# zrjer/Sparse-Matrix-Factorization-Library

Hardware: AMD Instinct MI355X
Metric: numeric-factorization GFLOP/s (supernodal Cholesky) (higher is better)
Workload: dtype f64; 1 GPU; 3D 7-point Laplacian 128^3 SPD Cholesky fp64, geometric ND, devSlotSize 8694792192; n=2097152, nnz_input=8339456, nsuper=35419, factor_doubles=3787034536, parallelism=single GPU, grid_rule=BASELINE config

## Files before the change

sparse-matrix-factorization-library_amd/csrc/sf_kernels.hip:

```cpp
#include "sf_kernels.h"
#include <cstdlib>
#include "sf_panel.h"
#include "sf_wave.h"

namespace sf {

__device__ __forceinline__ int lower_bound_i32(const int32_t* __restrict__ a, int n, int32_t key) {
    int lo = 0, hi = n;
    while (lo < hi) {
        const int mid = (lo + hi) >> 1;
        if (a[mid] < key) lo = mid + 1; else hi = mid;
    }
    return lo;
}

__global__ void __launch_bounds__(256)
k_load_panels(const int64_t* __restrict__ Lp, const int32_t* __restrict__ Li, const double* __restrict__ Lx, int32_t n,
              const int32_t* __restrict__ Super, const int32_t* __restrict__ SuperMap,
              const int64_t* __restrict__ Lsip, const int32_t* __restrict__ Lsi,
              const int64_t* __restrict__ Lsxp, double* __restrict__ Lsx, int skip_diag,
              const int8_t* __restrict__ load_mask) {
    const int32_t j = blockIdx.x * blockDim.x + threadIdx.x;
    if (j >= n) return;
    const int32_t s = SuperMap[j];
    if (load_mask && !load_mask[s]) return;
    const int32_t c0 = Super[s], c1 = Super[s + 1];
    const int64_t r0 = Lsip[s];
    const int32_t nsrow = (int32_t)(Lsip[s + 1] - r0);
    const int32_t nscol = c1 - c0;
    double* col = Lsx + Lsxp[s] + (int64_t)(j - c0) * nsrow;
    const int32_t* below = Lsi + r0 + nscol;
    for (int64_t p = Lp[j]; p < Lp[j + 1]; ++p) {
        const int32_t i = Li[p];
        if (skip_diag && i == j) continue;
        const int32_t si = (i < c1) ? (i - c0) : nscol + lower_bound_i32(below, nsrow - nscol, i);
        col[si] = Lx[p];
    }
}

__global__ void __launch_bounds__(256)
k_build_loadmap(const int64_t* __restrict__ Lp, const int32_t* __restrict__ Li, int32_t n,
                const int32_t* __restrict__ Super, const int32_t* __restrict__ SuperMap,
                const int64_t* __restrict__ Lsip, const int32_t* __restrict__ Lsi,
                const int64_t* __restrict__ Lsxp, int64_t base, int skip_diag, int64_t* __restrict__ map) {
    const int32_t j = blockIdx.x * blockDim.x + threadIdx.x;
    if (j >= n) return;
    const int32_t s = SuperMap[j];
    const int32_t c0 = Super[s], c1 = Super[s + 1];
    const int64_t r0 = Lsip[s];
    const int32_t nsrow = (int32_t)(Lsip[s + 1] - r0);
    const int32_t nscol = c1 - c0;
    const int64_t col = base + Lsxp[s] + (int64_t)(j - c0) * nsrow;
    const int32_t* below = Lsi + r0 + nscol;
    for (int64_t p = Lp[j]; p < Lp[j + 1]; ++p) {
        const int32_t i = Li[p];
        if (skip_diag && i == j) { map[p] = -1; continue; }
        const int32_t si = (i < c1) ? (i - c0) : nscol + lower_bound_i32(below, nsrow - nscol, i);
        map[p] = col + si;
    }
}

__global__ void __launch_bounds__(256)
k_load_mapped(const double* __restrict__ Lx, const int64_t* __restrict__ map, int64_t nnz, double* __restrict__ Lsx) {
    for (int64_t p = (int64_t)blockIdx.x * blockDim.x + threadIdx.x; p < nnz; p += (int64_t)gridDim.x * blockDim.x) {
        const int64_t m = map[p];
        if (m >= 0) Lsx[m] = Lx[p];
    }
}

__global__ void __launch_bounds__(256)
k_loadmap_drop(const int64_t* __restrict__ drop, int64_t count, int64_t* __restrict__ map) {
    for (int64_t k = (int64_t)blockIdx.x * blockDim.x + threadIdx.x; k < count; k += (int64_t)gridDim.x * blockDim.x) map[drop[k]] = -1;
}

void launch_loadmap_drop(const int64_t* drop, int64_t count, int64_t* map, hipStream_t st) {
    if (count <= 0) return;
    const int64_t blocks = std::min<int64_t>((count + 255) / 256, 1024);
    hipLaunchKernelGGL(k_loadmap_drop, dim3((unsigned)blocks), dim3(256), 0, st, drop, count, map);
}

void launch_build_loadmap(const int64_t* Lp, const int32_t* Li, int32_t n, const int32_t* Super, const int32_t* SuperMap,
                          const int64_t* Lsip, const int32_t* Lsi, const int64_t* Lsxp, int64_t base, int skip_diag, int64_t* map, hipStream_t st) {
    if (n <= 0) return;
    hipLaunchKernelGGL(k_build_loadmap, dim3((n + 255) / 256), dim3(256), 0, st, Lp, Li, n, Super, SuperMap, Lsip, Lsi, Lsxp, base, skip_diag, map);
}

void launch_load_mapped(const double* Lx, const int64_t* map, int64_t nnz, double* Lsx, hipStream_t st) {
    if (nnz <= 0) return;
    const int64_t blocks = std::min<int64_t>((nnz + 255) / 256, 256 * 16);
    hipLaunchKernelGGL(k_load_mapped, dim3((unsigned)blocks), dim3(256), 0, st, Lx, map, nnz, Lsx);
}

void launch_load_panels(const int64_t* Lp, const int32_t* Li, const double* Lx, int32_t n,
                        const int32_t* Super, const int32_t* SuperMap, const int64_t* Lsip, const int32_t* Lsi,
                        const int64_t* Lsxp, double* Lsx, int skip_diag, const int8_t* load_mask, hipStream_t st) {
    if (n <= 0) return;
    hipLaunchKernelGGL(k_load_panels, dim3((n + 255) / 256), dim3(256), 0, st,
                       Lp, Li, Lx, n, Super, SuperMap, Lsip, Lsi, Lsxp, Lsx, skip_diag, load_mask);
}

template <int W>
__device__ __forceinline__ void potrf_block_w(const PotrfTask& t, double* __restrict__ Lsx, int* __restrict__ info) {
    double* A = Lsx + t.panel + t.diag + (int64_t)t.diag * t.ld;
    const int b = t.b;
    const int lane = threadIdx.x;
    const int64_t ld = t.ld;

    double a[W];
#pragma unroll
    for (int c = 0; c < W; ++c) {
        double v = (c == lane) ? 1.0 : 0.0;
        if (lane < b && c <= lane) v = A[lane + c * ld];
        a[c] = v;
    }
    bool bad = false;
    double dnext = a[0];
#pragma unroll
    for (int j = 0; j < W; ++j) {
        const double djj = readlane_f64(dnext, j);
        bad = bad || !(djj > 0.0);
        const double rinv = rsqrt_full(djj);
        const double lj = a[j] * rinv;
        a[j] = lj;
        if (j + 1 < W) dnext = __builtin_fma(-lj, lj, a[j + 1]);
#pragma unroll
        for (int c = j + 1; c < W; ++c) a[c] = __builtin_fma(-lj, readlane_f64(lj, c), a[c]);
    }
    if (bad && lane == 0) atomicOr(info, 1);
#pragma unroll
    for (int c = 0; c < W; ++c)
        if (lane < b && c <= lane) A[lane + c * ld] = a[c];
}

__global__ void __launch_bounds__(64)
k_potrf_block(const PotrfTask* __restrict__ tasks, double* __restrict__ Lsx, int* __restrict__ info) {
    const PotrfTask t = tasks[blockIdx.x];
    if (t.b <= 8) potrf_block_w<8>(t, Lsx, info);
    else if (t.b <= 16) potrf_block_w<16>(t, Lsx, info);
    else if (t.b <= 32) potrf_block_w<32>(t, Lsx, info);
    else potrf_block_w<NB>(t, Lsx, info);
}

void launch_potrf(const PotrfTask* tasks, int ntasks, double* Lsx, int* info, hipStream_t st) {
    if (ntasks <= 0) return;
    hipLaunchKernelGGL(k_potrf_block, dim3(ntasks), dim3(64), 0, st, tasks, Lsx, info);
}

template <int W>
__device__ __forceinline__ void getrf_block_w(const PotrfTask& t, double* __restrict__ Lsx, int64_t u_shift, int* __restrict__ info, const PivotCtl& pc) {
    double* PLd = Lsx + t.panel + t.diag + (int64_t)t.diag * t.ld;
    double* PUd = PLd + u_shift;
    const int b = t.b;
    const int lane = threadIdx.x;
    const int64_t ld = t.ld;

    double a[W];
#pragma unroll
    for (int c = 0; c < W; ++c) {
        double v = (c == lane) ? 1.0 : 0.0;
        if (lane < b && c < b) v = (c < lane) ? PLd[lane + c * ld] : PUd[c + lane * ld];
        a[c] = v;
    }
    bool bad = false, active = lane < b;
    int np = 0, pos = lane;
    getrf_panel_wave<false, W>(a, lane, 0, b, pc.tol, pc.eps, bad, np, pos, active, nullptr);
    if (bad && lane == 0) atomicOr(info, 1);
    if (np > 0 && lane == 0) atomicAdd(pc.nperturb, np);
#pragma unroll
    for (int c = 0; c < W; ++c) {
        if (lane < b && c < b) {
            if (c < pos) PLd[pos + c * ld] = a[c]; else PUd[c + pos * ld] = a[c];
        }
    }
    if (pc.pivpos && lane < b) {
        const int g0 = t.first_col + t.diag;
        pc.pivpos[g0 + lane] = g0 + pos;
        pc.pivinv[g0 + pos] = g0 + lane;
    }
}

__global__ void __launch_bounds__(64)
k_getrf_block(const PotrfTask* __restrict__ tasks, double* __restrict__ Lsx, int64_t u_shift, int* __restrict__ info, PivotCtl pc) {
    const PotrfTask t = tasks[blockIdx.x];
    if (t.b <= 8) getrf_block_w<8>(t, Lsx, u_shift, info, pc);
    else if (t.b <= 16) getrf_block_w<16>(t, Lsx, u_shift, info, pc);
    else if (t.b <= 32) getrf_block_w<32>(t, Lsx, u_shift, info, pc);
    else getrf_block_w<NB>(t, Lsx, u_shift, info, pc);
}

void launch_getrf(const PotrfTask* tasks, int ntasks, double* Lsx, int64_t u_shift, int* info, PivotCtl pc, hipStream_t st) {
    if (ntasks <= 0) return;
    hipLaunchKernelGGL(k_getrf_block, dim3(ntasks), dim3(64), 0, st, tasks, Lsx, u_shift, info, pc);
}

__global__ void __launch_bounds__(256)
k_pack_lu(const int32_t* __restrict__ Super, const int64_t* __restrict__ Lsip, const int64_t* __restrict__ Xp,
          const int64_t* __restrict__ RefXp, int32_t nsuper, const double* __restrict__ PL, const double* __restrict__ PU,
          double* __restrict__ out, int64_t e_begin, int64_t e_end) {
    for (int64_t e = e_begin + (int64_t)blockIdx.x * blockDim.x + threadIdx.x; e < e_end; e += (int64_t)gridDim.x * blockDim.x) {
        double* __restrict__ dst = out + (e - e_begin);
        int lo = 0, hi = nsuper;
        while (hi - lo > 1) {
            const int mid = (lo + hi) >> 1;
            if (RefXp[mid] <= e) lo = mid; else hi = mid;
        }
        const int s = lo;
        if (Xp[s] < 0) { *dst = 0.0; continue; }
        const int64_t nscol = Super[s + 1] - Super[s], nsrow = Lsip[s + 1] - Lsip[s];
        const int64_t lda = 2 * nsrow - nscol;
        const int64_t off = e - RefXp[s];
        const int64_t j = off / lda, R = off % lda;
        const double* pl = PL + Xp[s] + j * nsrow;
        double v;
        if (R < nscol) v = (R > j) ? pl[R] : PU[Xp[s] + j + R * nsrow];
        else if (R < nsrow) v = pl[R];
        else v = PU[Xp[s] + (R - nsrow + nscol) + j * nsrow];
        *dst = v;
    }
}

void launch_pack_lu(const int32_t* Super, const int64_t* Lsip, const int64_t* Xp, const int64_t* RefXp, int32_t nsuper,
                    const double* PL, const double* PU, double* out, int64_t e_begin, int64_t e_end, hipStream_t st) {
    if (e_end <= e_begin) return;
    const int64_t blocks = (e_end - e_begin + 255) / 256;
    hipLaunchKernelGGL(k_pack_lu, dim3((unsigned)(blocks < 65536 ? blocks : 65536)), dim3(256), 0, st,
                       Super, Lsip, Xp, RefXp, nsuper, PL, PU, out, e_begin, e_end);
}

__global__ void __launch_bounds__(256)
k_factor_hash(const int32_t* __restrict__ Super, const int64_t* __restrict__ Lsip, const int64_t* __restrict__ Xp,
              const int64_t* __restrict__ RefXp, int32_t nsuper, const double* __restrict__ PL, const double* __restrict__ PU, int lu,
              int64_t total, int64_t chunk, unsigned long long* __restrict__ H) {
    const int64_t begin = (int64_t)blockIdx.x * chunk, end = min(begin + chunk, total);
    if (begin >= end) return;
    const bool idle = begin + threadIdx.x >= end;
    int64_t e = idle ? end - 1 : begin + threadIdx.x;
    int lo = 0, hi = nsuper;
    while (hi - lo > 1) {
        const int mid = (lo + hi) >> 1;
        if (RefXp[mid] <= e) lo = mid; else hi = mid;
    }
    int s = lo;
    unsigned long long acc = 0;
    int64_t s_end = RefXp[s + 1], s_beg = RefXp[s], xp = Xp[s];
    int64_t nscol = Super[s + 1] - Super[s], nsrow = Lsip[s + 1] - Lsip[s];
    if (idle) e = end;
    for (; e < end; e += 256) {
        if (e >= s_end) {
            if (acc) atomicAdd(&H[s], acc);
            acc = 0;
            while (e >= RefXp[s + 1]) ++s;
            s_end = RefXp[s + 1]; s_beg = RefXp[s]; xp = Xp[s];
            nscol = Super[s + 1] - Super[s]; nsrow = Lsip[s + 1] - Lsip[s];
        }
        if (xp < 0) {
            e += ((s_end - e + 255) / 256 - 1) * 256;
            continue;
        }
        const int64_t off = e - s_beg;
        double v;
        if (!lu) {
            v = PL[xp + off];
        } else {
            const int64_t lda = 2 * nsrow - nscol;
            const int64_t j = off / lda, R = off % lda;
            if (R < nscol) v = (R > j) ? PL[xp + j * nsrow + R] : PU[xp + j + R * nsrow];
            else if (R < nsrow) v = PL[xp + j * nsrow + R];
            else v = PU[xp + (R - nsrow + nscol) + j * nsrow];
        }
        acc += (unsigned long long)__double_as_longlong(v) * ((2ull * (unsigned long long)e + 1ull) * 0x9E3779B97F4A7C15ull);
    }
    __shared__ int s_first;
    __shared__ unsigned long long s_part[4];
    if (threadIdx.x == 0) s_first = s;
    __syncthreads();
    const bool uniform = __syncthreads_and(s == s_first) != 0;
    if (!uniform) { if (acc) atomicAdd(&H[s], acc); return; }
    for (int off = 32; off > 0; off >>= 1) acc += __shfl_down(acc, off, 64);
    if ((threadIdx.x & 63) == 0) s_part[threadIdx.x >> 6] = acc;
    __syncthreads();
    if (threadIdx.x == 0) {
        const unsigned long long tot = s_part[0] + s_part[1] + s_part[2] + s_part[3];
        if (tot) atomicAdd(&H[s], tot);
    }
}

void launch_factor_hash(const int32_t* Super, const int64_t* Lsip, const int64_t* Xp, const int64_t* RefXp, int32_t nsuper,
                        const double* PL, const double* PU, int lu, int64_t total, unsigned long long* H, hipStream_t st) {
    if (total <= 0 || nsuper <= 0) return;
    const int64_t chunk = 256 * 64;
    const int64_t blocks = (total + chunk - 1) / chunk;
    hipLaunchKernelGGL(k_factor_hash, dim3((unsigned)blocks), dim3(256), 0, st, Super, Lsip, Xp, RefXp, nsuper, PL, PU, lu, total, chunk, H);
}

__global__ void __launch_bounds__(256)
k_lu_fill_u11(const FillTile* __restrict__ tiles, double* __restrict__ PL, const double* __restrict__ PU) {
    __shared__ double tile[64][65];
    const FillTile t = tiles[blockIdx.x];
    const int tx = threadIdx.x & 63, ty = threadIdx.x >> 6;
    const int jlo = max(t.c0, t.cb), jhi = min(t.c0 + 64, t.ce);
    {
        const int j = t.c0 + tx;
        for (int rr = ty; rr < 64; rr += 4) {
            const int R = t.r0 + rr;
            if (j >= jlo && j < jhi && R <= j) tile[rr][tx] = PU[t.xp + j + (int64_t)R * t.nsrow];
        }
    }
    __syncthreads();
    {
        const int R = t.r0 + tx;
        for (int jj = ty; jj < 64; jj += 4) {
            const int j = t.c0 + jj;
            if (j >= jlo && j < jhi && R <= j) PL[t.xp + R + (int64_t)j * t.nsrow] = tile[tx][jj];
        }
    }
}

void launch_lu_fill_u11(const FillTile* tiles, int64_t ntiles, double* PL, const double* PU, hipStream_t st) {
    if (ntiles <= 0) return;
    hipLaunchKernelGGL(k_lu_fill_u11, dim3((unsigned)ntiles), dim3(256), 0, st, tiles, PL, PU);
}

__global__ void __launch_bounds__(TRSM_ROWS)
k_trsm_block(const TrsmTask* __restrict__ tasks, double* __restrict__ Lsx, const int32_t* __restrict__ pivinv) {
    __shared__ __attribute__((aligned(16))) double Dt[NB][NB];
    __shared__ double Dinv[NB];
    const TrsmTask t = tasks[blockIdx.x];
    const double* Dg = Lsx + t.dpanel + t.diag + (int64_t)t.diag * t.ld;
    const int b = t.b;
    const int tid = threadIdx.x;

    for (int e = tid; e < b * NB; e += (int)blockDim.x) {
        const int k = e / NB, j = e % NB;
        Dt[k][j] = (j < b && k < j) ? Dg[j + (int64_t)k * t.ld] : 0.0;
    }
    if (tid < NB) Dinv[tid] = (tid < b && !t.unit) ? 1.0 / Dg[tid + (int64_t)tid * t.ld] : 1.0;
    __syncthreads();

    if (tid >= t.nrows) return;
    double* X = Lsx + t.panel + t.row0 + tid + (int64_t)t.diag * t.ld;
    const int64_t ld = t.ld;
    if (pivinv && t.unit) {
        const int g0 = t.first_col + t.diag;
        const int32_t* pv = pivinv + g0;
        double tmp[NB];
#pragma unroll
        for (int c = 0; c < NB; ++c) tmp[c] = X[(int64_t)(pv[min(c, b - 1)] - g0) * ld];
#pragma unroll
        for (int c = 0; c < NB; ++c)
            if (c < b) X[(int64_t)c * ld] = tmp[c];
    }

    for (int jb = 0; jb < b; jb += 8) {
        double acc[8];
#pragma unroll
        for (int u = 0; u < 8; ++u) acc[u] = X[min(jb + u, b - 1) * ld];
#pragma unroll
        for (int u = 0; u < 8; ++u) acc[u] = (jb + u < b) ? acc[u] : 0.0;
        for (int k0 = 0; k0 < jb; k0 += 8) {
            double xk[8];
#pragma unroll
            for (int v = 0; v < 8; ++v) xk[v] = X[(k0 + v) * ld];
#pragma unroll
            for (int v = 0; v < 8; ++v)
#pragma unroll
                for (int u = 0; u < 8; ++u) acc[u] -= xk[v] * Dt[k0 + v][jb + u];
        }
#pragma unroll
        for (int u = 0; u < 8; ++u) {
#pragma unroll
            for (int v = 0; v < u; ++v) acc[u] -= acc[v] * Dt[jb + v][jb + u];
            acc[u] *= Dinv[jb + u];
        }
#pragma unroll
        for (int u = 0; u < 8; ++u)
            if (jb + u < b) X[(jb + u) * ld] = acc[u];
    }
}

void launch_trsm(const TrsmTask* tasks, int ntasks, double* Lsx, const int32_t* pivinv, hipStream_t st) {
    if (ntasks <= 0) return;
    hipLaunchKernelGGL(k_trsm_block, dim3(ntasks), dim3(TRSM_ROWS), 0, st, tasks, Lsx, pivinv);
}

constexpr int LDS_LD = GEMM_BM + 16;
constexpr int GEMM_SK = GEMM_BK / 2;
#ifndef SF_GEMM_MIN_UNITS_DEFAULT
#define SF_GEMM_MIN_UNITS_DEFAULT 16
#endif

__device__ __forceinline__ int last_le_u32(const uint32_t* __restrict__ a, int n, uint32_t key) {
    int lo = 0, hi = n;
    while (hi - lo > 1) {
        const int mid = (lo + hi) >> 1;
        if (a[mid] <= key) lo = mid; else hi = mid;
    }
    return lo;
}

__device__ double g_zero_page[GEMM_BM + 16];

__device__ __forceinline__ void glds16(const void* sbase, uint32_t voff, uint32_t lds_dst) {
    unsigned keep;
    asm volatile("s_mov_b32 %0, m0\n\ts_mov_b32 m0, %3\n\ts_nop 0\n\tglobal_load_lds_dwordx4 %2, %1\n\ts_mov_b32 m0, %0"
                 : "=&s"(keep) : "s"(sbase), "v"(voff), "s"(lds_dst) : "memory");
}
__device__ __forceinline__ uint32_t lds_addr(const void* p) {
    return __builtin_amdgcn_readfirstlane((uint32_t)(uintptr_t)(__attribute__((address_space(3))) const void*)p);
}

#ifdef SF_EXP_TIMING
__device__ unsigned long long* g_exp_stamps = nullptr;
void exp_set_stamps(unsigned long long* p) { (void)hipMemcpyToSymbol(HIP_SYMBOL(g_exp_stamps), &p, sizeof(p)); }
#define SF_STAMP(slot) do { if (tid == 0 && g_exp_stamps && exp_tile < 64) \
        g_exp_stamps[((size_t)blockIdx.x * 64 + exp_tile) * 4 + (slot)] = __builtin_amdgcn_s_memtime(); } while (0)
#else
#define SF_STAMP(slot) do { } while (0)
#endif

template <int MODE, bool DMA>
__global__ void __launch_bounds__(GEMM_THREADS, GEMM_WAVES / 2)
k_gemm(const GemmProb* __restrict__ probs, const GemmTask* __restrict__ tasks,
       const uint32_t* __restrict__ kt_prefix, int ntasks, uint32_t u_lo, uint32_t u_hi,
       double* __restrict__ Lsx, const int32_t* __restrict__ RelMap, int* __restrict__ ticket, int whole_tiles, uint32_t min_units) {
    __shared__ int s_claim;
    __shared__ __attribute__((aligned(16))) double Ys[2][GEMM_BK][LDS_LD];
    __shared__ __attribute__((aligned(16))) double Xs[2][GEMM_BK][LDS_LD];
    __shared__ int32_t rowmap[GEMM_BM];
    __shared__ int32_t colmap[GEMM_BN];

    constexpr int WCJ = GEMM_BN / (GEMM_WAVES / 2);
    constexpr int TMN = WCJ / 16;
    constexpr int SQ = GEMM_BK / GEMM_WAVES;
    const int tid = threadIdx.x;
    const int lane = tid & 63, wave = tid >> 6;
    const int wm = wave & 1, wn = wave >> 1;
    const int fr = lane & 15, fk = lane >> 4;
    const int swave = __builtin_amdgcn_readfirstlane(wave);
    const uint32_t lds_ys = lds_addr(&Ys[0][0][0]), lds_xs = lds_addr(&Xs[0][0][0]);

    const uint32_t T = u_hi - u_lo;
    const uint32_t G = gridDim.x;
    const uint32_t xcd = blockIdx.x & 7;
    const uint32_t xcd_n = (G >> 3) + (xcd < (G & 7) ? 1u : 0u);
    const uint32_t xcd_base = xcd < (G & 7) ? xcd * ((G >> 3) + 1) : (G & 7) * ((G >> 3) + 1) + (xcd - (G & 7)) * (G >> 3);
    const uint32_t share = xcd_base + (blockIdx.x >> 3);
    (void)T;
    int t0 = last_le_u32(kt_prefix, ntasks + 1, u_lo);
    if (kt_prefix[t0] < u_lo) ++t0;
    const int t1 = last_le_u32(kt_prefix, ntasks + 1, u_hi);
    const int R = (t1 > t0) ? (int)(((uint32_t)(t1 - t0) + (whole_tiles ? G - 1 : 0)) / G) : 0;
    const uint32_t head_end = (R > 0) ? kt_prefix[t0] : u_hi;
    const uint32_t tail_beg = (R > 0 && !whole_tiles) ? kt_prefix[t0 + R * (int)G] : u_hi;

    int ph = 0, rr = 0;
#ifdef SF_EXP_DEPHASE
    bool exp_dephased = false;
#endif
#ifdef SF_EXP_TIMING
    int exp_tile = 0;
    if (tid == 0 && g_exp_stamps) {
        g_exp_stamps[(size_t)gridDim.x * 256 + blockIdx.x * 4 + 0] = __builtin_amdgcn_s_memtime();
        g_exp_stamps[(size_t)gridDim.x * 256 + blockIdx.x * 4 + 1] = wall_clock64();
    }
#endif
    for (;;) {
    uint32_t u, u_end;
    int ti;
    SF_STAMP(0);
    if (ph == 1) {
        uint32_t slot = share;
        if (ticket != nullptr && R > 0) {
            if (tid == 0) s_claim = __hip_atomic_fetch_add(ticket + xcd, 1, __ATOMIC_RELAXED, __HIP_MEMORY_SCOPE_AGENT);
            __syncthreads();
            const uint32_t c = (uint32_t)__builtin_amdgcn_readfirstlane(s_claim);
            rr = (int)(c / xcd_n);
            slot = xcd_base + c % xcd_n;
        }
        if (rr >= R) { ph = 2; continue; }
        ti = t0 + rr * (int)G + (int)slot;
        ++rr;
        if (ti >= t1) continue;
        u = kt_prefix[ti];
        u_end = kt_prefix[ti + 1];
#ifdef SF_EXP_DEPHASE
        if (!exp_dephased && blockIdx.x >= gridDim.x / 2) {
            const int naps = (int)(u_end - u) * SF_EXP_DEPHASE / 16;
            for (int i = 0; i < naps; ++i) __builtin_amdgcn_s_sleep(127);
        }
        exp_dephased = true;
#endif
    } else {
        const uint32_t ra = (ph == 0) ? u_lo : tail_beg, rb = (ph == 0) ? head_end : u_hi;
        const uint32_t Ueq = (rb > ra) ? (rb - ra + G - 1) / G : 0, U = max(Ueq, min_units);
        const uint32_t sh = (U > Ueq) ? blockIdx.x : share;
        if (rb <= ra || sh * U >= rb - ra) {
            if (ph == 0) { ph = 1; continue; }
            break;
        }
        u = ra + sh * U;
        u_end = min(rb, u + U);
        ti = last_le_u32(kt_prefix, ntasks + 1, u);
    }

    while (u < u_end) {
        const GemmTask tk = tasks[ti];
        const GemmProb pb = probs[tk.prob];
        const uint32_t tbase = kt_prefix[ti];
        const int nkt = (int)(kt_prefix[ti + 1] - tbase);
        const int kt0 = (int)(u - tbase);
        const int kt1 = min(nkt, kt0 + (int)(u_end - u));
        u += (uint32_t)(kt1 - kt0);
        ++ti;

        const int ci0 = tk.tm * GEMM_BM, cj0 = tk.tn * GEMM_BN;
        const int M = pb.M, N = pb.N;
        const int lda = pb.lda;
        const int kfirst = (int)tk.kt0 * GEMM_BK;
        const int K = min(pb.K - kfirst, nkt * GEMM_BK);
        const double* __restrict__ Yg = Lsx + pb.y_off + ci0 + (int64_t)kfirst * lda;
        const double* __restrict__ Xg = Lsx + pb.x_off + cj0 + (int64_t)kfirst * lda;

        if (MODE == 1) {
            if (tid < GEMM_BM) {
                const int ci = ci0 + tid;
                rowmap[tid] = (ci < M) ? RelMap[pb.map_off + ci] : 0;
            } else if (tid < GEMM_BM + GEMM_BN) {
                const int cj = cj0 + (tid - GEMM_BM);
                colmap[tid - GEMM_BM] = (cj < N) ? RelMap[pb.map_off + cj] : 0;
            }
        }

        const int prow = 2 * (tid & 63), pk0 = tid >> 6;
        const bool y0_ok = (ci0 + prow) < M, y1_ok = (ci0 + prow + 1) < M;
        const bool x0_ok = (cj0 + prow) < N, x1_ok = (cj0 + prow + 1) < N;
        const double* __restrict__ yp = Yg + (y0_ok ? prow : 0);
        const double* __restrict__ xp = Xg + (x0_ok ? prow : 0);
        const uint32_t yoff = (y0_ok ? prow : 0) * (uint32_t)sizeof(double), xoff = (x0_ok ? prow : 0) * (uint32_t)sizeof(double);
        double2_t ry[DMA ? 1 : SQ], rx[DMA ? 1 : SQ];

        auto load_tile = [&](int k0) {
#pragma unroll
            for (int q = 0; q < SQ; ++q) {
                const int64_t off = (int64_t)min(k0 + pk0 + GEMM_WAVES * q, K - 1) * lda;
                ry[q] = *reinterpret_cast<const double2_t*>(yp + off);
                rx[q] = *reinterpret_cast<const double2_t*>(xp + off);
            }
        };
        auto store_tile = [&](int buf, int k0) {
#pragma unroll
            for (int q = 0; q < SQ; ++q) {
                const bool kin = (k0 + pk0 + GEMM_WAVES * q) < K;
                double2_t vy = ry[q], vx = rx[q];
                vy.x = (kin && y0_ok) ? vy.x : 0.0; vy.y = (kin && y1_ok) ? vy.y : 0.0;
                vx.x = (kin && x0_ok) ? vx.x : 0.0; vx.y = (kin && x1_ok) ? vx.y : 0.0;
                *reinterpret_cast<double2_t*>(&Ys[buf][pk0 + GEMM_WAVES * q][prow]) = vy;
                *reinterpret_cast<double2_t*>(&Xs[buf][pk0 + GEMM_WAVES * q][prow]) = vx;
            }
        };
        auto dma_stage = [&](int buf, int half, int kt) {
            const int kl = half * GEMM_SK + swave, k = kt * GEMM_BK + kl;
            const uint32_t slot = (uint32_t)((buf * GEMM_BK + kl) * LDS_LD) * (uint32_t)sizeof(double);
            const bool kin = k < K;
            const double* ysrc = Yg + (int64_t)min(k, K - 1) * lda;
            const double* xsrc = kin ? Xg + (int64_t)k * lda : g_zero_page;
            glds16(ysrc, yoff, lds_ys + slot);
            glds16(xsrc, xoff, lds_xs + slot);
        };
        auto read_frag = [&](double (&a)[TMN], double (&b)[4], int buf, int krow) {
#pragma unroll
            for (int t = 0; t < TMN; ++t) a[t] = Xs[buf][krow + fk][wn * WCJ + t * 16 + fr];
#pragma unroll
            for (int t = 0; t < 4; ++t) b[t] = Ys[buf][krow + fk][wm * 64 + t * 16 + fr];
        };

        const int qci0 = ci0 + wm * 64, qcj0 = cj0 + wn * WCJ;
        const bool quad_active = __builtin_amdgcn_readfirstlane((int)((qci0 < M) && (qcj0 < N) && (qci0 + 63 >= qcj0))) != 0;

        double4_t acc[TMN][4];
#pragma unroll
        for (int a = 0; a < TMN; ++a)
#pragma unroll
            for (int b = 0; b < 4; ++b) acc[a][b] = (double4_t){0.0, 0.0, 0.0, 0.0};

        auto mma = [&](const double (&a)[TMN], const double (&b)[4]) {
#pragma unroll
            for (int tm = 0; tm < TMN; ++tm)
#pragma unroll
                for (int tn = 0; tn < 4; ++tn)
                    acc[tm][tn] = __builtin_amdgcn_mfma_f64_16x16x4f64(a[tm], b[tn], acc[tm][tn], 0, 0, 0);
        };

        if constexpr (DMA) {
        dma_stage(0, 0, kt0);
        dma_stage(0, 1, kt0);
        if (kt0 + 1 < kt1) {
            dma_stage(1, 0, kt0 + 1);
            asm volatile("s_waitcnt vmcnt(2)" ::: "memory");
        } else {
            asm volatile("s_waitcnt vmcnt(0)" ::: "memory");
        }
        __syncthreads();
        SF_STAMP(1);
        if (quad_active) {
            double a0[TMN], b0[4], a1[TMN], b1[4];
            read_frag(a0, b0, 0, 0);
            auto k_step = [&](const int buf, int kt) {
#pragma unroll
                for (int h = 0; h < 2; ++h) {
                    const bool more = kt + 1 + h < kt1;
                    read_frag(a1, b1, buf, h * GEMM_SK + 4);
                    if (more) dma_stage(h ? buf : buf ^ 1, h ^ 1, kt + 1 + h);
                    mma(a0, b0);
                    read_frag(a0, b0, h ? buf ^ 1 : buf, h ? 0 : GEMM_SK);
                    mma(a1, b1);
                    if (more) asm volatile("s_waitcnt vmcnt(2)" ::: "memory");
                    else asm volatile("s_waitcnt vmcnt(0)" ::: "memory");
                    __syncthreads();
                }
            };
            int kt = kt0;
            for (; kt + 1 < kt1; kt += 2) {
                k_step(0, kt);
                k_step(1, kt + 1);
            }
            if (kt < kt1) k_step(0, kt);
        } else {
            for (int kt = kt0; kt < kt1; ++kt) {
                const int buf = (kt - kt0) & 1;
#pragma unroll
                for (int h = 0; h < 2; ++h) {
                    if (kt + 1 + h < kt1) {
                        dma_stage(h ? buf : buf ^ 1, h ^ 1, kt + 1 + h);
                        asm volatile("s_waitcnt vmcnt(2)" ::: "memory");
                    } else {
                        asm volatile("s_waitcnt vmcnt(0)" ::: "memory");
                    }
                    __syncthreads();
                }
            }
        }
        } else {
        load_tile(kt0 * GEMM_BK);
        store_tile(0, kt0 * GEMM_BK);
        __syncthreads();
        SF_STAMP(1);
        load_tile((kt0 + 1) * GEMM_BK);
        int buf = 0;
        if (quad_active) {
            for (int kt = kt0; kt < kt1; ++kt) {
#pragma unroll
                for (int kk = 0; kk < GEMM_BK / 4; ++kk) {
                    double a[TMN], b[4];
                    read_frag(a, b, buf, kk * 4);
                    if (kk == 0) store_tile(buf ^ 1, (kt + 1) * GEMM_BK);
                    if (kk == 1) load_tile((kt + 2) * GEMM_BK);
                    mma(a, b);
                }
                __syncthreads();
                buf ^= 1;
            }
        } else {
            for (int kt = kt0; kt < kt1; ++kt) {
                store_tile(buf ^ 1, (kt + 1) * GEMM_BK);
                load_tile((kt + 2) * GEMM_BK);
                __syncthreads();
                buf ^= 1;
            }
        }
        }

        SF_STAMP(2);
#ifdef SF_EXP_SKIP_EPILOGUE
        if (quad_active) {
            double v = 0.0;
            for (int tm = 0; tm < TMN; ++tm) for (int tn = 0; tn < 4; ++tn) for (int r = 0; r < 4; ++r) v += acc[tm][tn][r];
            if (v == 12345.678) Lsx[pb.c_off] = v;
        }
#else
        if (quad_active) {
            double* __restrict__ Cg = Lsx + pb.c_off;
            const int64_t ldc = pb.ldc;
#pragma unroll
            for (int tm = 0; tm < TMN; ++tm) {
#pragma unroll
                for (int tn = 0; tn < 4; ++tn) {
                    const int lci = wm * 64 + tn * 16 + fr;
                    const int ci = ci0 + lci;
#pragma unroll
                    for (int r = 0; r < 4; ++r) {
                        const int lcj = wn * WCJ + tm * 16 + fk + 4 * r;
                        const int cj = cj0 + lcj;
                        if (ci < M && cj < N && ci >= cj + (pb.strict & 1)) {
                            const double v = acc[tm][tn][r];
                            if (MODE == 1) {
                                unsafeAtomicAdd(Cg + rowmap[lci] + (int64_t)colmap[lcj] * ldc, -v);
                            } else {
                                double* dst = Cg + ci + (int64_t)cj * ldc;
                                unsafeAtomicAdd(dst, -v);
                            }
                        }
                    }
                }
            }
        }
#endif
        __syncthreads();
        SF_STAMP(3);
#ifdef SF_EXP_TIMING
        ++exp_tile;
        SF_STAMP(0);
#endif
    }
    if (ph == 2) break;
    if (ph == 0) ph = 1;
    }
#ifdef SF_EXP_TIMING
    if (tid == 0 && g_exp_stamps) {
        g_exp_stamps[(size_t)gridDim.x * 256 + blockIdx.x * 4 + 2] = __builtin_amdgcn_s_memtime();
        g_exp_stamps[(size_t)gridDim.x * 256 + blockIdx.x * 4 + 3] = wall_clock64();
    }
#endif
}

__global__ void __launch_bounds__(256)
k_update_small(const GemmProb* __restrict__ probs, const GemmTask* __restrict__ tasks, int ntasks,
               double* __restrict__ Lsx, const int32_t* __restrict__ RelMap) {
    const int lane = threadIdx.x & 63;
    const int ti = __builtin_amdgcn_readfirstlane(blockIdx.x * 4 + (threadIdx.x >> 6));
    if (ti >= ntasks) return;
    const GemmTask tk = tasks[ti];
    const GemmProb pb = probs[tk.prob];
    const int fr = lane & 15, fk = lane >> 4;
    const int ci0 = tk.tm * SU_TM, cj0 = tk.tn * SU_TN;
    const int M = pb.M, N = pb.N, K = pb.K;
    const int64_t lda = pb.lda;
    const double* __restrict__ yq[4];
    const double* __restrict__ xq[2];
#pragma unroll
    for (int q = 0; q < 4; ++q) yq[q] = Lsx + pb.y_off + min(ci0 + 16 * q + fr, M - 1);
#pragma unroll
    for (int q = 0; q < 2; ++q) xq[q] = Lsx + pb.x_off + min(cj0 + 16 * q + fr, N - 1);

    double4_t acc[2][4];
#pragma unroll
    for (int a = 0; a < 2; ++a)
#pragma unroll
        for (int c = 0; c < 4; ++c) acc[a][c] = (double4_t){0.0, 0.0, 0.0, 0.0};

    const int nkk = (K + 3) >> 2;
    for (int kk0 = 0; kk0 < nkk; kk0 += 8) {
        double fa[8][2], fb[8][4];
#pragma unroll
        for (int kk = 0; kk < 8; ++kk) {
            const int k = 4 * (kk0 + kk) + fk;
            const int64_t off = (int64_t)min(k, K - 1) * lda;
#pragma unroll
            for (int q = 0; q < 2; ++q) fa[kk][q] = xq[q][off];
#pragma unroll
            for (int q = 0; q < 4; ++q) fb[kk][q] = yq[q][off];
#pragma unroll
            for (int q = 0; q < 2; ++q) fa[kk][q] = (k < K) ? fa[kk][q] : 0.0;
        }
#pragma unroll
        for (int kk = 0; kk < 8; ++kk) {
            if (kk0 + kk < nkk) {
#pragma unroll
                for (int tm = 0; tm < 2; ++tm)
#pragma unroll
                    for (int tn = 0; tn < 4; ++tn)
                        acc[tm][tn] = __builtin_amdgcn_mfma_f64_16x16x4f64(fa[kk][tm], fb[kk][tn], acc[tm][tn], 0, 0, 0);
            }
        }
    }

    double* __restrict__ Cg = Lsx + pb.c_off;
    const int64_t ldc = pb.ldc;
    const int32_t* __restrict__ rm = RelMap + pb.map_off;
    int32_t colm[2][4];
#pragma unroll
    for (int tm = 0; tm < 2; ++tm)
#pragma unroll
        for (int r = 0; r < 4; ++r) colm[tm][r] = rm[min(cj0 + 16 * tm + fk + 4 * r, N - 1)];
#pragma unroll
    for (int tn = 0; tn < 4; ++tn) {
        const int ci = ci0 + 16 * tn + fr;
        const int32_t rowm = rm[min(ci, M - 1)];
#pragma unroll
        for (int tm = 0; tm < 2; ++tm)
#pragma unroll
            for (int r = 0; r < 4; ++r) {
                const int cj = cj0 + 16 * tm + fk + 4 * r;
                if (ci < M && cj < N && ci >= cj + (pb.strict & 1))
                    unsafeAtomicAdd(Cg + rowm + (int64_t)colm[tm][r] * ldc, -acc[tm][tn][r]);
            }
    }
}

void launch_update_small(const GemmProb* probs, const GemmTask* tasks, int ntasks, double* Lsx, const int32_t* RelMap, hipStream_t st) {
    if (ntasks <= 0) return;
    hipLaunchKernelGGL(k_update_small, dim3((ntasks + 3) / 4), dim3(256), 0, st, probs, tasks, ntasks, Lsx, RelMap);
}

__global__ void __launch_bounds__(256)
k_resid_init(int32_t n, double* __restrict__ r, double* __restrict__ colsum, double* __restrict__ b_out) {
    const int32_t i = blockIdx.x * blockDim.x + threadIdx.x;
    if (i >= n) return;
    const double b = 1.0 + (double)i / (double)n;
    b_out[i] = b;
    r[i] = -b;
    colsum[i] = 0.0;
}

__global__ void __launch_bounds__(256)
k_resid_cols(const int64_t* __restrict__ Lp, const int32_t* __restrict__ Li, const double* __restrict__ Lx, int32_t n, int sym,
             const double* __restrict__ x, double* __restrict__ r, double* __restrict__ colsum) {
    const int32_t j = blockIdx.x * blockDim.x + threadIdx.x;
    if (j >= n) return;
    const double xj = x[j];
    double rj = 0.0, cj = 0.0;
    for (int64_t p = Lp[j]; p < Lp[j + 1]; ++p) {
        const int32_t i = Li[p];
        const double a = Lx[p];
        unsafeAtomicAdd(r + i, a * xj);
        cj += fabs(a);
        if (sym && i != j) {
            rj += a * x[i];
            unsafeAtomicAdd(colsum + i, fabs(a));
        }
    }
    if (rj != 0.0) unsafeAtomicAdd(r + j, rj);
    unsafeAtomicAdd(colsum + j, cj);
}

__global__ void __launch_bounds__(256)
k_resid_urows(const int64_t* __restrict__ Up, const int32_t* __restrict__ Ui, const double* __restrict__ Ux, int32_t n,
              const double* __restrict__ x, double* __restrict__ r, double* __restrict__ colsum) {
    const int32_t i = blockIdx.x * blockDim.x + threadIdx.x;
    if (i >= n) return;
    double ri = 0.0;
    for (int64_t p = Up[i]; p < Up[i + 1]; ++p) {
        const int32_t j = Ui[p];
        if (j == i) continue;
        ri += Ux[p] * x[j];
        unsafeAtomicAdd(colsum + j, fabs(Ux[p]));
    }
    if (ri != 0.0) unsafeAtomicAdd(r + i, ri);
}

__global__ void __launch_bounds__(256)
k_resid_norms(int32_t n, const double* __restrict__ r, const double* __restrict__ colsum, const double* __restrict__ x,
              const double* __restrict__ b, unsigned long long* __restrict__ norms) {
    double m[4] = {0.0, 0.0, 0.0, 0.0};
    for (int32_t i = blockIdx.x * blockDim.x + threadIdx.x; i < n; i += gridDim.x * blockDim.x) {
        m[0] = fmax(m[0], fabs(r[i])); m[1] = fmax(m[1], colsum[i]); m[2] = fmax(m[2], fabs(x[i])); m[3] = fmax(m[3], fabs(b[i]));
    }
#pragma unroll
    for (int k = 0; k < 4; ++k) {
        double v = m[k];
#pragma unroll
        for (int off = 32; off > 0; off >>= 1) v = fmax(v, __shfl_down(v, off, 64));
        if ((threadIdx.x & 63) == 0) atomicMax(norms + k, (unsigned long long)__double_as_longlong(v));
    }
}

__global__ void k_noop() {}
void launch_noop(hipStream_t st) { hipLaunchKernelGGL(k_noop, dim3(1), dim3(64), 0, st); }

void launch_residual(const int64_t* Lp, const int32_t* Li, const double* Lx, const int64_t* Up, const int32_t* Ui, const double* Ux,
                     int32_t n, const double* x, double* r, double* colsum, double* b, double* norms, hipStream_t st) {
    if (n <= 0) return;
    const int g = (n + 255) / 256;
    hipLaunchKernelGGL(k_resid_init, dim3(g), dim3(256), 0, st, n, r, colsum, b);
    hipLaunchKernelGGL(k_resid_cols, dim3(g), dim3(256), 0, st, Lp, Li, Lx, n, Up ? 0 : 1, x, r, colsum);
    if (Up) hipLaunchKernelGGL(k_resid_urows, dim3(g), dim3(256), 0, st, Up, Ui, Ux, n, x, r, colsum);
    hipLaunchKernelGGL(k_resid_norms, dim3(g < 1024 ? g : 1024), dim3(256), 0, st, n, r, colsum, x, b, (unsigned long long*)norms);
}

__global__ void __launch_bounds__(256)
k_build_relmaps(const GemmProb* __restrict__ probs, const int32_t* __restrict__ Lsi, int32_t* __restrict__ RelMap) {
    const GemmProb pb = probs[blockIdx.x];
    for (int ci = threadIdx.x; ci < pb.M; ci += blockDim.x) {
        const int32_t g = Lsi[pb.src_rows + ci];
        RelMap[pb.map_off + ci] = (ci < pb.N) ? (g - pb.tgt_first_col)
                                              : pb.tgt_nscol + lower_bound_i32(Lsi + pb.tgt_rows, pb.tgt_nbelow, g);
    }
}

void launch_build_relmaps(const GemmProb* probs, int nprobs, const int32_t* Lsi, int32_t* RelMap, hipStream_t st) {
    if (nprobs > 0) hipLaunchKernelGGL(k_build_relmaps, dim3(nprobs), dim3(256), 0, st, probs, Lsi, RelMap);
}

void launch_gemm(const GemmProb* probs, const GemmTask* tasks, const uint32_t* kt_prefix, int ntasks, uint32_t u_lo, uint32_t u_hi,
                 int mode, double* Lsx, const int32_t* RelMap, int* ticket, hipStream_t st, int whole_tiles, int grid_cap) {
    if (ntasks <= 0 || u_hi <= u_lo) return;
    const uint32_t units = u_hi - u_lo;
    const uint32_t cap = (grid_cap > 0 && grid_cap < GEMM_GRID) ? (uint32_t)grid_cap : (uint32_t)GEMM_GRID;
    const uint32_t grid = units < cap ? units : cap;
    static const uint32_t min_units = [] { const char* m = getenv("SF_GEMM_MIN_UNITS"); return (uint32_t)(m ? std::max(1, atoi(m)) : SF_GEMM_MIN_UNITS_DEFAULT); }();
    const char* e = sf_exp_env("SF_GEMM_DMA");
    const bool dma = e ? atoi(e) != 0 : true;
    if (dma) {
        if (mode == 1)
            hipLaunchKernelGGL((k_gemm<1, true>), dim3(grid), dim3(GEMM_THREADS), 0, st, probs, tasks, kt_prefix, ntasks, u_lo, u_hi, Lsx, RelMap, ticket, whole_tiles, min_units);
        else
            hipLaunchKernelGGL((k_gemm<0, true>), dim3(grid), dim3(GEMM_THREADS), 0, st, probs, tasks, kt_prefix, ntasks, u_lo, u_hi, Lsx, RelMap, ticket, whole_tiles, min_units);
        return;
    }
    if (mode == 1)
        hipLaunchKernelGGL((k_gemm<1, false>), dim3(grid), dim3(GEMM_THREADS), 0, st, probs, tasks, kt_prefix, ntasks, u_lo, u_hi, Lsx, RelMap, ticket, whole_tiles, min_units);
    else
        hipLaunchKernelGGL((k_gemm<0, false>), dim3(grid), dim3(GEMM_THREADS), 0, st, probs, tasks, kt_prefix, ntasks, u_lo, u_hi, Lsx, RelMap, ticket, whole_tiles, min_units);
}

}
```

Measured before the change: 55810 GFLOP/s.

## Prefetch next GEMM task descriptors and pre-claim work tickets during current tile

In the GEMM kernel's persistent loop, the atomic ticket claim for the next tile is issued at the start of the current tile and published through a double-buffered shared slot. The next task's descriptor and prefix bounds are prefetched during the mainloop, and its problem descriptor after it, so the following tile starts without dependent global loads. The RelMap loads are hoisted into registers and written to LDS later, overlapping them with the first DMA stage. This targets per-tile setup latency, the atomic plus barrier round-trip, at the cost of more registers and more complex control flow, with a possible occupancy loss.

```diff
diff --git a/sparse-matrix-factorization-library_amd/csrc/sf_kernels.hip b/sparse-matrix-factorization-library_amd/csrc/sf_kernels.hip
--- a/sparse-matrix-factorization-library_amd/csrc/sf_kernels.hip
+++ b/sparse-matrix-factorization-library_amd/csrc/sf_kernels.hip
@@ -409,13 +409,32 @@
     return __builtin_amdgcn_readfirstlane((uint32_t)(uintptr_t)(__attribute__((address_space(3))) const void*)p);
 }
 
+__device__ __forceinline__ int opaque_lane_zero() {
+    int z;
+    asm("v_mov_b32 %0, 0" : "=v"(z));
+    return z;
+}
+template <class T>
+__device__ __forceinline__ T to_scalar(const T& v) {
+    static_assert(sizeof(T) % 4 == 0, "dword-wise");
+    uint32_t w[sizeof(T) / 4];
+    __builtin_memcpy(w, &v, sizeof(T));
+#pragma unroll
+    for (size_t i = 0; i < sizeof(T) / 4; ++i) w[i] = (uint32_t)__builtin_amdgcn_readfirstlane((int)w[i]);
+    T r;
+    __builtin_memcpy(&r, w, sizeof(T));
+    return r;
+}
+
 #ifdef SF_EXP_TIMING
 __device__ unsigned long long* g_exp_stamps = nullptr;
 void exp_set_stamps(unsigned long long* p) { (void)hipMemcpyToSymbol(HIP_SYMBOL(g_exp_stamps), &p, sizeof(p)); }
 #define SF_STAMP(slot) do { if (tid == 0 && g_exp_stamps && exp_tile < 64) \
-        g_exp_stamps[((size_t)blockIdx.x * 64 + exp_tile) * 4 + (slot)] = __builtin_amdgcn_s_memtime(); } while (0)
+        g_exp_stamps[((size_t)blockIdx.x * 64 + exp_tile) * 8 + (slot)] = __builtin_amdgcn_s_memtime(); } while (0)
+#define SF_STAMP_LANDED(slot) do { asm volatile("s_waitcnt vmcnt(0) lgkmcnt(0)" ::: "memory"); SF_STAMP(slot); } while (0)
 #else
 #define SF_STAMP(slot) do { } while (0)
+#define SF_STAMP_LANDED(slot) do { } while (0)
 #endif
 
 template <int MODE, bool DMA>
@@ -423,7 +442,7 @@
 k_gemm(const GemmProb* __restrict__ probs, const GemmTask* __restrict__ tasks,
        const uint32_t* __restrict__ kt_prefix, int ntasks, uint32_t u_lo, uint32_t u_hi,
        double* __restrict__ Lsx, const int32_t* __restrict__ RelMap, int* __restrict__ ticket, int whole_tiles, uint32_t min_units) {
-    __shared__ int s_claim;
+    __shared__ int s_claim[2];
     __shared__ __attribute__((aligned(16))) double Ys[2][GEMM_BK][LDS_LD];
     __shared__ __attribute__((aligned(16))) double Xs[2][GEMM_BK][LDS_LD];
     __shared__ int32_t rowmap[GEMM_BM];
@@ -454,14 +473,20 @@
     const uint32_t tail_beg = (R > 0 && !whole_tiles) ? kt_prefix[t0 + R * (int)G] : u_hi;
 
     int ph = 0, rr = 0;
+    int cpar = 0;
+    bool have_claim = false;
+    int nx_ti = -1;
+    GemmTask nx_tk{};
+    GemmProb nx_pb{};
+    uint32_t nx_p0 = 0, nx_p1 = 0;
 #ifdef SF_EXP_DEPHASE
     bool exp_dephased = false;
 #endif
 #ifdef SF_EXP_TIMING
     int exp_tile = 0;
     if (tid == 0 && g_exp_stamps) {
-        g_exp_stamps[(size_t)gridDim.x * 256 + blockIdx.x * 4 + 0] = __builtin_amdgcn_s_memtime();
-        g_exp_stamps[(size_t)gridDim.x * 256 + blockIdx.x * 4 + 1] = wall_clock64();
+        g_exp_stamps[(size_t)gridDim.x * 512 + blockIdx.x * 4 + 0] = __builtin_amdgcn_s_memtime();
+        g_exp_stamps[(size_t)gridDim.x * 512 + blockIdx.x * 4 + 1] = wall_clock64();
     }
 #endif
     for (;;) {
@@ -471,9 +496,13 @@
     if (ph == 1) {
         uint32_t slot = share;
         if (ticket != nullptr && R > 0) {
-            if (tid == 0) s_claim = __hip_atomic_fetch_add(ticket + xcd, 1, __ATOMIC_RELAXED, __HIP_MEMORY_SCOPE_AGENT);
-            __syncthreads();
-            const uint32_t c = (uint32_t)__builtin_amdgcn_readfirstlane(s_claim);
+            if (!have_claim) {
+                if (tid == 0) s_claim[cpar] = __hip_atomic_fetch_add(ticket + xcd, 1, __ATOMIC_RELAXED, __HIP_MEMORY_SCOPE_AGENT);
+                __syncthreads();
+            }
+            const uint32_t c = (uint32_t)__builtin_amdgcn_readfirstlane(s_claim[cpar]);
+            cpar ^= 1;
+            have_claim = false;
             rr = (int)(c / xcd_n);
             slot = xcd_base + c % xcd_n;
         }
@@ -503,11 +532,24 @@
         ti = last_le_u32(kt_prefix, ntasks + 1, u);
     }
 
+    SF_STAMP(4);
     while (u < u_end) {
-        const GemmTask tk = tasks[ti];
-        const GemmProb pb = probs[tk.prob];
-        const uint32_t tbase = kt_prefix[ti];
-        const int nkt = (int)(kt_prefix[ti + 1] - tbase);
+        const bool preclaim = (ph == 1 && ticket != nullptr);
+        int nclaim = 0;
+        if (preclaim && tid == 0) nclaim = __hip_atomic_fetch_add(ticket + xcd, 1, __ATOMIC_RELAXED, __HIP_MEMORY_SCOPE_AGENT);
+        GemmTask tk;
+        GemmProb pb;
+        uint32_t tbase, tnext;
+        if (nx_ti == ti) {
+            tk = to_scalar(nx_tk); pb = to_scalar(nx_pb); tbase = to_scalar(nx_p0); tnext = to_scalar(nx_p1);
+        } else {
+            tk = tasks[ti];
+            pb = probs[tk.prob];
+            tbase = kt_prefix[ti];
+            tnext = kt_prefix[ti + 1];
+        }
+        SF_STAMP_LANDED(5);
+        const int nkt = (int)(tnext - tbase);
         const int kt0 = (int)(u - tbase);
         const int kt1 = min(nkt, kt0 + (int)(u_end - u));
         u += (uint32_t)(kt1 - kt0);
@@ -521,15 +563,32 @@
         const double* __restrict__ Yg = Lsx + pb.y_off + ci0 + (int64_t)kfirst * lda;
         const double* __restrict__ Xg = Lsx + pb.x_off + cj0 + (int64_t)kfirst * lda;
 
-        if (MODE == 1) {
-            if (tid < GEMM_BM) {
-                const int ci = ci0 + tid;
-                rowmap[tid] = (ci < M) ? RelMap[pb.map_off + ci] : 0;
-            } else if (tid < GEMM_BM + GEMM_BN) {
-                const int cj = cj0 + (tid - GEMM_BM);
-                colmap[tid - GEMM_BM] = (cj < N) ? RelMap[pb.map_off + cj] : 0;
-            }
-        }
+        int32_t mapv = 0;
+        if (MODE == 1 && tid < GEMM_BM + GEMM_BN) {
+            const int c = (tid < GEMM_BM) ? ci0 + tid : cj0 + (tid - GEMM_BM);
+            if (c < ((tid < GEMM_BM) ? M : N)) mapv = RelMap[pb.map_off + c];
+        }
+        auto publish = [&]() {
+            if (MODE == 1) {
+                if (tid < GEMM_BM) rowmap[tid] = mapv;
+                else if (tid < GEMM_BM + GEMM_BN) colmap[tid - GEMM_BM] = mapv;
+            }
+            if (preclaim && tid == 0) s_claim[cpar] = nclaim;
+        };
+        auto next_tile = [&]() -> int {
+            if (u < u_end) return ti;
+            if (ph != 1) return -1;
+            int r2 = rr;
+            uint32_t slot2 = share;
+            if (preclaim) {
+                const uint32_t c = (uint32_t)__builtin_amdgcn_readfirstlane(s_claim[cpar]);
+                r2 = (int)(c / xcd_n);
+                slot2 = xcd_base + c % xcd_n;
+            }
+            if (r2 >= R) return -1;
+            const int p = t0 + r2 * (int)G + (int)slot2;
+            return p < t1 ? p : -1;
+        };
 
         const int prow = 2 * (tid & 63), pk0 = tid >> 6;
         const bool y0_ok = (ci0 + prow) < M, y1_ok = (ci0 + prow + 1) < M;
@@ -591,17 +650,25 @@
                     acc[tm][tn] = __builtin_amdgcn_mfma_f64_16x16x4f64(a[tm], b[tn], acc[tm][tn], 0, 0, 0);
         };
 
+        int pred = -1;
         if constexpr (DMA) {
         dma_stage(0, 0, kt0);
         dma_stage(0, 1, kt0);
         if (kt0 + 1 < kt1) {
             dma_stage(1, 0, kt0 + 1);
+            publish();
+            SF_STAMP(6);
             asm volatile("s_waitcnt vmcnt(2)" ::: "memory");
         } else {
+            publish();
+            SF_STAMP(6);
             asm volatile("s_waitcnt vmcnt(0)" ::: "memory");
         }
         __syncthreads();
         SF_STAMP(1);
+        pred = next_tile();
+        const int pv = max(pred, 0) + opaque_lane_zero();
+        nx_tk = tasks[pv]; nx_p0 = kt_prefix[pv]; nx_p1 = kt_prefix[pv + 1];
         if (quad_active) {
             double a0[TMN], b0[4], a1[TMN], b1[4];
             read_frag(a0, b0, 0, 0);
@@ -643,6 +710,8 @@
         } else {
         load_tile(kt0 * GEMM_BK);
         store_tile(0, kt0 * GEMM_BK);
+        publish();
+        SF_STAMP(6);
         __syncthreads();
         SF_STAMP(1);
         load_tile((kt0 + 1) * GEMM_BK);
@@ -671,6 +740,9 @@
         }
 
         SF_STAMP(2);
+        if constexpr (DMA) nx_pb = probs[nx_tk.prob];
+        nx_ti = pred;
+        if (preclaim) have_claim = true;
 #ifdef SF_EXP_SKIP_EPILOGUE
         if (quad_active) {
             double v = 0.0;
@@ -717,8 +789,8 @@
     }
 #ifdef SF_EXP_TIMING
     if (tid == 0 && g_exp_stamps) {
-        g_exp_stamps[(size_t)gridDim.x * 256 + blockIdx.x * 4 + 2] = __builtin_amdgcn_s_memtime();
-        g_exp_stamps[(size_t)gridDim.x * 256 + blockIdx.x * 4 + 3] = wall_clock64();
+        g_exp_stamps[(size_t)gridDim.x * 512 + blockIdx.x * 4 + 2] = __builtin_amdgcn_s_memtime();
+        g_exp_stamps[(size_t)gridDim.x * 512 + blockIdx.x * 4 + 3] = wall_clock64();
     }
 #endif
 }
```

Result: no change. 55440 GFLOP/s (-0.7%).
